# oss0430/SRFRD

Measured on AMD Instinct MI355X. Metric: sequences/sec, higher is better.
Workload: dtype f32

## Files before the change

srfrd_amd/csrc/srfrd_encoder_bwd_ragged_kernel.inc:

```
namespace SRFRD_NS {


struct RagBwdLds {
  lds_f* base;
  lds_f* s_ln;
  lds_f* s_lng;
};

template <int K_, int DI_, bool RMW_>
__device__ __forceinline__ void rag_bwd_seq(const EncArgs& a, const RagBwdLds& m, int b, int iter, int& tid, int wave, uint32_t seed) {
  const Dims& ly = a.dm;
  constexpr int nw = 8, nthr = 512;
  constexpr int L = 50, D = 50, LP = 64, DK = 52, DS = 54, NT = 4, MT = 4;
  constexpr int R = 52, SZ = R * DS, SLD = R + 2, SH = kRagSH;
  static_assert(SH == LP - R && R * SLD <= SZ + 2 * R, "slot geometry");
  static_assert(kRagBwdWork == SH * DS + 6 * SZ + 13 * LP, "working set");
  constexpr bool CV2 = true;
  constexpr int CIT = (R * (D / 2) + nthr - 1) / nthr;
  constexpr int PIT = (R * (R / 2) + nthr - 1) / nthr;
  lds_f* slot[6];
#pragma unroll
  for (int s = 0; s < 6; ++s) slot[s] = m.base + SH * DS + s * SZ;
  lds_f* tail = m.base + SH * DS + 6 * SZ;
  lds_i* s_in = (lds_i*)tail;
  lds_f* s_keep = tail + LP;
  lds_i* s_pid = (lds_i*)(tail + 2 * LP);
  lds_i* s_nid = (lds_i*)(tail + 3 * LP);
  lds_i* s_fk = (lds_i*)(tail + 4 * LP);
  lds_i* s_pfk = (lds_i*)(tail + 5 * LP);
  lds_i* s_nfk = (lds_i*)(tail + 6 * LP);
  lds_f* s_dpl = tail + 7 * LP;
  lds_f* s_dnl = tail + 8 * LP;
  lds_f* s_delta = tail + 9 * LP;
  lds_f* s_brep = tail + 10 * LP;
  lds_f* s_dummy = tail + 11 * LP;
  lds_f* s_misc = tail + 12 * LP;
  lds_f* s_ln = m.s_ln;
  lds_f* s_lng = m.s_lng;
  const float* P = a.dense;
  const bool drop_on = a.drop_on != 0;
  const int rkind = K_ >= 0 ? K_ : ly.kind;
  const bool is_sas = rkind == SRFRD_SASREC;
  const bool has_fake = rkind == SRFRD_SRFR || rkind == SRFRD_SRFRN;
  const bool is_srfu = rkind >= SRFRD_SRFU_B;
  constexpr int di = DI_, dfk = D - DI_;
  constexpr int dout = (K_ == SRFRD_SRFR) ? DI_ : D;
  const float sqrtD = sqrtf((float)di);
  const float qscale = a.qscale;
  const int B = a.B;
  auto pk = [&](int mat, int form) {
    return PackedB{reinterpret_cast<const float4*>(a.packed) + ((int64_t)mat * 2 + form) * (kPackFloats / 4)};
  };
  static_assert(L <= nthr && (R - L) * DS <= nthr, "single-pass helpers");
  auto ones_col = [&](lds_f* buf) {
    if (tid < L) buf[tid * DS + D] = 1.0f;
  };
  auto zero_pad_rows = [&](lds_f* buf) {
    if (tid < (R - L) * DS) buf[L * DS + tid] = 0.f;
  };
  const float keep_scale = drop_on ? a.drop_scale : 1.0f;

  asm volatile("" : "+v"(tid));
  float* slab = a.grad_slabs + (int64_t)blockIdx.x * ly.n_dense;
  const int rmw = RMW_ ? (iter != 0) : 0;
  if (iter == 0)
    for (int i = tid; i < ly.blk0; i += nthr) slab[i] = 0.f;
  const int64_t rowbase = (int64_t)b * L;
  const uint32_t seq = (uint32_t)(a.seq0 + b);
  const int lane0 = tid & 63;
  if (tid < LP) {
    const int t = tid;
    const bool in = t < L;
    const int id = in ? clamp_id(a.in_ids[rowbase + t], ly.n_items) : 0;
    const int pid = (in && a.pos_ids) ? clamp_id(a.pos_ids[rowbase + t], ly.n_items) : 0;
    const int nid = (in && a.neg_ids) ? clamp_id(a.neg_ids[rowbase + t], ly.n_items) : 0;
    s_in[t] = id;
    s_keep[t] = id != 0 ? 1.f : 0.f;
    s_pid[t] = pid;
    s_nid[t] = nid;
    s_fk[t] = (in && a.fk_ids) ? clamp_id(a.fk_ids[rowbase + t], 2) : 0;
    s_pfk[t] = (in && a.pos_fk) ? clamp_id(a.pos_fk[rowbase + t], 2) : 0;
    s_nfk[t] = (in && a.neg_fk) ? clamp_id(a.neg_fk[rowbase + t], 2) : 0;
    float dp = 0.f, dn = 0.f;
    if (in) {
      if (a.fused_bce) {
        const float pl = a.c_pl[rowbase + t], nl = a.c_nl[rowbase + t];
        if (pid != 0) {
          dp = sigmoid_f(pl) - 1.0f;
          dn = sigmoid_f(nl);
        }
      } else {
        if (a.d_pos && a.pos_ids) dp = a.d_pos[rowbase + t];
        if (a.d_neg && a.neg_ids) dn = a.d_neg[rowbase + t];
      }
    }
    s_dpl[t] = dp;
    s_dnl[t] = dn;
  }
  if (is_srfu && wave == 1) {
    const int lab = user_label_wave(rkind, a.fk_ids ? a.fk_ids + rowbase : nullptr, L, ly.n_labels);
    if (lane0 == 0) ((lds_i*)s_misc)[0] = lab;
  }
  __syncthreads();
  int t0, th;
  {
    const bool inr = lane0 < L;
    const unsigned long long nz = __ballot(inr && s_in[lane0] != 0);
    const unsigned long long ng = __ballot(inr && (s_in[lane0] != 0 || s_dpl[lane0] != 0.f || s_dnl[lane0] != 0.f));
    t0 = nz ? (int)__builtin_ctzll(nz) : L;
    th = ng ? (int)__builtin_ctzll(ng) : L;
    if (a.ragged_off) t0 = 0;
    if (a.d_hidden != nullptr || a.ragged_off) th = 0;
    t0 = __builtin_amdgcn_readfirstlane(t0);
    th = __builtin_amdgcn_readfirstlane(th);
  }
  const int krp = t0 >= 1 ? t0 - 1 : 0;
  const int kr = krp + SH, v0 = t0 + SH;
  const int mt0 = kr >> 4, r0 = mt0 << 4, mtn = MT - mt0;
  const int p0 = r0 > SH ? r0 - SH : 0;
  const int k0 = p0 + SH;
  const int hp = th < krp ? th : krp;
  const int mh0 = (hp + SH) >> 4, rh0 = mh0 << 4, mhn = MT - mh0;
  const int ph0 = rh0 > SH ? rh0 - SH : 0, kh0 = ph0 + SH;

  lds_f *sX = slot[0], *sQ = slot[1], *sG = slot[2], *sT = slot[3], *sK = slot[4], *sO = slot[5];
  lds_f* dummy = s_dummy;
#define TB(p) ((p) - SH * DS)
  G2L<CIT, CV2> g_last, g_h1, g_r;
  g_last.load(a.c_save_x + x_off(ly.n_blocks, b, ly.n_blocks, L, D) + p0 * D, L - p0, D, nthr);
  g_h1.load(a.c_save_h1 + h1_off(ly.n_blocks - 1, b, ly.n_blocks, L, D) + p0 * D, L - p0, D, nthr);
  g_r.load(a.c_save_aux + aux_off(ly.n_blocks - 1, b, ly.n_blocks, L, LP, D).r + p0 * D, L - p0, D, nthr);
  g_last.store(sX + p0 * DS, DS, L - p0, D, nthr);
  for (int r = ph0 + (tid >> 6); r < p0; r += nthr >> 6) {
    const int c = tid & 63;
    if (c < DS && c != D) sX[r * DS + c] = 0.f;
  }
  zero_pad_rows(sX);
  ones_col(sX);
  zero_pad_rows(sG);
  __syncthreads();

  int lane = tid & 63, li = lane & 15, lq = lane >> 4;
#define RG_RELANE() do { asm volatile("" : "+v"(tid)); lane = tid & 63; li = lane & 15; lq = lane >> 4; } while (0)
  const int nt_w = wave & 3, g_w = wave >> 2;
  auto slab_gemm = [&](int kk0, auto amat, auto bmat, const SlabWB& sl, const SlabPre& pre) {
    f32x4 acc[2];
#pragma unroll
    for (int j = 0; j < 2; ++j) acc[j] = f32x4{pre.v[j][0], pre.v[j][1], pre.v[j][2], pre.v[j][3]};
    mma_group<2>(acc, amat, bmat, (g_w << 4) + li, 32, (nt_w << 4) + li, kk0, LP, lq);
    const SlabCol sc = slab_col(sl, (nt_w << 4) + li);
    if (sc.ok) {
#pragma unroll
      for (int j = 0; j < 2; ++j)
#pragma unroll
        for (int e = 0; e < 4; ++e) {
          const int r = ((g_w + 2 * j) << 4) + (lq << 2) + e;
          if (r < sl.R) sl.base[(unsigned)(sc.col0 + r * sc.rs)] = acc[j][e];
        }
    }
  };
  auto col_sums = [&](int kk0, const lds_f* m_b, lds_f* dst, int ncol) {
    if (wave < NT) {
      f32x4 acc[1] = {f32x4{0.f, 0.f, 0.f, 0.f}};
      mma_group<1>(acc, OnesRow{}, Mat{m_b, DS}, li, 0, (wave << 4) + li, kk0, LP, lq);
      const int c = (wave << 4) + li;
      if (lq == 0 && c < ncol) dst[c] += acc[0][0];
    }
  };
  auto side_sums = [&](int n_out, auto term, auto dst_off, int tlo) {
    for (int p = wave; p < n_out; p += nw) {
      float sacc = 0.f;
      for (int t = tlo + lane; t < L; t += 64) sacc += term(p, t);
      sacc = wave_sum(sacc);
      if (lane == 0) atomicAdd(&slab[dst_off(p)], sacc);
    }
  };

  const lds_f* lnin = sX;
  if (K_ == SRFRD_SRFR) {
    const WFrag wl = load_wfrag(pk(ly.n_blocks * 6, 0), P + ly.off_lc_b, di, (di + 15) >> 4, tid);
    {
      constexpr int nst = (di + 15) >> 4;
      const int nt3 = wave % nst, g3 = wave / nst;
      auto epi = [&](int r, int c, float v) { *((c < di && r >= SH && r < SH + L) ? &TB(sQ)[r * DS + c] : dummy + c) = v; };
      if (g3 < 2) {
        if (g3 + 2 < mhn) gemm_group_packed<2>(mh0 + g3, 2, nt3, DK >> 2, Mat{TB(sX), DS}, wl, epi, lane);
        else if (g3 < mhn) gemm_group_packed<1>(mh0 + g3, 2, nt3, DK >> 2, Mat{TB(sX), DS}, wl, epi, lane);
      }
    }
    __syncthreads();
    lnin = sQ;
  }
  {
    const bool srfrn = K_ == SRFRD_SRFRN;
    const int n = (L - ph0) * dout;
    constexpr int GIT = (LP * D + nthr - 1) / nthr;
    constexpr int HALF = (GIT + 1) / 2;
    const float* hid = a.c_hidden + (rowbase + ph0) * dout;
    const float* dhid = a.d_hidden ? a.d_hidden + (rowbase + ph0) * dout : nullptr;
    int tg = tid;
    asm volatile("" : "+v"(tg));
    auto chunks = [&](auto bf16_shadow) {
      constexpr bool H16 = decltype(bf16_shadow)::value;
      for (int base0 = 0; base0 < n; base0 += HALF * nthr) {
        float hv[HALF], pv[HALF], nv[HALF];
#pragma unroll
        for (int u = 0; u < HALF; ++u) {
          const int i = min(base0 + u * nthr + tg, n - 1);
          const int tt = i / dout, c = i - tt * dout, t = ph0 + tt;
          const bool item = c < di;
          const int prow = item ? s_pid[t] : s_pfk[t], nrow = item ? s_nid[t] : s_nfk[t];
          const int w = item ? di : dfk, cc = item ? c : c - di;
          const bool use = item || srfrn;
          hv[u] = hid[i];
          if constexpr (H16) {
            const float* side = P + ly.off_side;
            const float ps = side[(use && !item) ? prow * dfk + cc : 0], ns = side[(use && !item) ? nrow * dfk + cc : 0];
            const uint16_t ph = a.table16[item ? (int64_t)prow * di + cc : 0], nh = a.table16[item ? (int64_t)nrow * di + cc : 0];
            pv[u] = item ? bf16_to_f32(ph) : ps;
            nv[u] = item ? bf16_to_f32(nh) : ns;
          } else {
            const float* src = item ? a.table : P + ly.off_side;
            pv[u] = src[use ? (int64_t)prow * w + cc : 0];
            nv[u] = src[use ? (int64_t)nrow * w + cc : 0];
          }
        }
#pragma unroll
        for (int u = 0; u < HALF; ++u) {
          const int i = base0 + u * nthr + tg;
          if (i < n) {
            const int tt = i / dout, c = i - tt * dout, t = ph0 + tt;
            float dh = dhid ? dhid[i] : 0.f;
            if (c < di || srfrn) dh += s_dpl[t] * pv[u] + s_dnl[t] * nv[u];
            sT[t * DS + c] = hv[u];
            sG[t * DS + c] = dh;
          }
        }
      }
    };
    if (a.table16 != nullptr) chunks(std::true_type{});
    else chunks(std::false_type{});
    if (dout < D)
      for (int idx = tid; idx < (L - ph0) * (D - dout); idx += nthr) {
        const int tt = idx / (D - dout), cc = dout + idx - tt * (D - dout);
        sG[(ph0 + tt) * DS + cc] = 0.f;
      }
  }
  __syncthreads();
  {
    int t = ph0 + tid / di, c = tid - (tid / di) * di;
    constexpr int dt = nthr / di, dc = nthr - dt * di;
    for (; t < L;) {
      const float h = sT[t * DS + c];
      const float dp = s_dpl[t], dn = s_dnl[t];
      const int pid = s_pid[t], nid = s_nid[t];
      if (a.contrib != nullptr) {
        a.contrib[(((int64_t)0 * B + b) * L + t) * di + c] = pid != 0 ? dp * h : 0.f;
        a.contrib[(((int64_t)1 * B + b) * L + t) * di + c] = nid != 0 ? dn * h : 0.f;
      } else {
        if (pid != 0 && dp != 0.f) atomicAdd(&a.grad_table[(int64_t)pid * di + c], dp * h);
        if (nid != 0 && dn != 0.f) atomicAdd(&a.grad_table[(int64_t)nid * di + c], dn * h);
      }
      t += dt; c += dc;
      if (c >= di) { c -= di; ++t; }
    }
    if (a.contrib != nullptr)
      for (int idx = tid; idx < ph0 * di; idx += nthr) {
        a.contrib[(((int64_t)0 * B + b) * L) * di + idx] = 0.f;
        a.contrib[(((int64_t)1 * B + b) * L) * di + idx] = 0.f;
      }
  }
  if (K_ == SRFRD_SRFRN)
    side_sums(2 * dfk, [&](int p, int t) {
      constexpr int dq = dfk > 0 ? dfk : 1;
      const int f = 1 + p / dq, c = p - (f - 1) * dq;
      const float w = (s_pfk[t] == f ? s_dpl[t] : 0.f) + (s_nfk[t] == f ? s_dnl[t] : 0.f);
      return w * sT[t * DS + di + c];
    }, [&](int p) { return ly.off_side + dfk + p; }, ph0);
  ln_bwd_rows<false>(nw, sG + ph0 * DS, lnin + ph0 * DS, sK + ph0 * DS, sO + ph0 * DS, L - ph0, R - ph0, DS, dout,
                     s_ln + (4 * ly.n_blocks) * 64);
  if (dout < D)
    for (int idx = tid; idx < (L - ph0) * (D - dout); idx += nthr) {
      const int tt = idx / (D - dout), cc = dout + idx - tt * (D - dout);
      sK[(ph0 + tt) * DS + cc] = 0.f;
    }
  zero_pad_rows(sK);
  __syncthreads();
  col_sums(kh0, TB(sG), s_lng + (4 * ly.n_blocks + 1) * 64, dout);
  col_sums(kh0, TB(sO), s_lng + (4 * ly.n_blocks + 0) * 64, dout);
  __syncthreads();
  lds_f* G = sK;
  lds_f* fr[5] = {sG, sO, sT, sQ, sX};
  if (K_ == SRFRD_SRFR) {
    {
      const SlabWB sl{slab, ly.off_lc_w, ly.off_lc_b, di, D, rmw};
      SlabPre pre = RMW_ ? slab_preload(nw, NT, NT, sl) : SlabPre{};
      slab_gemm(kh0, MatT{TB(G), DS}, Mat{TB(sX), DS}, sl, pre);
    }
    const WFrag wln = load_wfrag(pk(ly.n_blocks * 6, 1), nullptr, 0, NT, tid);
    lds_f* Gn = sG;
    {
      auto epi = [&](int r, int c, float v) { *((c < D && r >= SH) ? &TB(Gn)[r * DS + c] : dummy + c) = v; };
      if (g_w + 2 < mhn) gemm_group_packed<2>(mh0 + g_w, 2, nt_w, ((di + 3) & ~3) >> 2, Mat{TB(G), DS}, wln, epi, lane);
      else if (g_w < mhn) gemm_group_packed<1>(mh0 + g_w, 2, nt_w, ((di + 3) & ~3) >> 2, Mat{TB(G), DS}, wln, epi, lane);
    }
    __syncthreads();
    fr[0] = G;
    G = Gn;
  }

  for (int i = ly.n_blocks - 1; i >= 0; --i) {
    const BlkOff o = blk_off(ly.blk0 + i * ly.blk_stride, D);
    const DropSite ds2 = drop_site(drop_on, seed, site_ffn2(i), seq, a.drop_thr, a.drop_scale);
    const AuxOff ax = aux_off(i, b, ly.n_blocks, L, LP, D);
    RG_RELANE();
    lds_f *X = fr[0], *Rr = fr[1], *N = fr[2], *A2 = fr[3], *A1 = fr[4];
    launder(G); launder(X); launder(Rr); launder(N); launder(A2); launder(A1);
    const WFrag w2n = load_wfrag(pk(i * 6 + 5, 1), nullptr, 0, NT, tid);
    const SlabWB sl_w2{slab, o.c2_w, o.c2_b, D, D, rmw};
    const SlabWB sl_w1{slab, o.c1_w, o.c1_b, D, D, rmw};
    {
      const int c = tid & 63;
      if (c < D)
        for (int r = p0 + (tid >> 6); r < R; r += nthr >> 6) {
          const float g = r < L ? G[r * DS + c] * s_keep[r] : 0.f;
          if (r < L) G[r * DS + c] = g;
          A2[r * DS + c] = g * drop_mul(ds2, r, c);
        }
    }
    g_h1.store(X + p0 * DS, DS, L - p0, D, nthr);
    g_r.store(Rr + p0 * DS, DS, L - p0, D, nthr);
    zero_pad_rows(X); zero_pad_rows(Rr); zero_pad_rows(G);
    ones_col(Rr);
    __syncthreads();
    ln_rows(nw, X + p0 * DS, N + p0 * DS, L - p0, DS, D, s_ln + (4 * i + 2) * 64, s_ln + (4 * i + 3) * 64);
    zero_pad_rows(N);
    ones_col(N);
    __syncthreads();
    G2L<CIT, CV2> g_o, g_v, g_k;
    {
      SlabPre pre_w2 = RMW_ ? slab_preload(nw, NT, NT, sl_w2) : SlabPre{};
      rag_packed(mt0, mtn, DK >> 2, D, Mat{TB(A2), DS}, w2n, [&](int r, int c) { return TB(Rr)[r * DS + c]; },
                 [&](int r, int c, float v, float act) {
        *(r >= SH ? &TB(A1)[r * DS + c] : dummy + c) = act > 0.f ? v * keep_scale : 0.f;
      }, lane, wave);
      slab_gemm(k0, MatT{TB(A2), DS}, Mat{TB(Rr), DS}, sl_w2, pre_w2);
    }
    const WFrag w1n = load_wfrag(pk(i * 6 + 4, 1), nullptr, 0, NT, tid);
    g_o.load(a.c_save_aux + ax.o + p0 * D, L - p0, D, nthr);
    __syncthreads();
    {
      SlabPre pre_w1 = RMW_ ? slab_preload(nw, NT, NT, sl_w1) : SlabPre{};
      rag_packed(mt0, mtn, DK >> 2, D, Mat{TB(A1), DS}, w1n, [&](int r, int c) { return TB(G)[r * DS + c]; },
                 [&](int r, int c, float v, float old) { *(r >= SH ? &TB(G)[r * DS + c] : dummy + c) = old + v; }, lane, wave);
      slab_gemm(k0, MatT{TB(A1), DS}, Mat{TB(N), DS}, sl_w1, pre_w1);
    }
    g_v.load(a.c_save_aux + ax.v + p0 * D, L - p0, D, nthr);
    __syncthreads();
    lds_f *H = A2, *GX = Rr;
    ln_bwd_rows<false>(nw, G + p0 * DS, X + p0 * DS, H + p0 * DS, GX + p0 * DS, L - p0, R - p0, DS, D, s_ln + (4 * i + 2) * 64);
    zero_pad_rows(H);
    g_k.load(a.c_save_aux + ax.k + p0 * D, L - p0, D, nthr);
    __syncthreads();
    lds_f* O = N;
    col_sums(k0, TB(G), s_lng + (4 * i + 3) * 64, D);
    col_sums(k0, TB(GX), s_lng + (4 * i + 2) * 64, D);
    g_o.store(O + p0 * DS, DS, L - p0, D, nthr);
    zero_pad_rows(O);
    ones_col(O);
    const WFrag won = load_wfrag(pk(i * 6 + 3, 1), nullptr, 0, NT, tid);
    G2L<PIT, true> g_p;
    g_p.load2d(a.c_save_aux + ax.p + p0 * LP + p0, L - p0, R - p0, LP, nthr);
    float brep_v = 0.f;
    if (tid < L && tid >= t0 && t0 >= 1) brep_v = a.c_save_aux[ax.p + tid * LP + LP - 1];
    __syncthreads();
    lds_f *DO = G, *V = GX, *Kk = X, *S = A1;
    RG_RELANE();
    const SlabWB sl_wo{slab, o.out_w, o.out_b, D, D, rmw};
    G2L<CIT, CV2> g_q, g_x;
    {
      SlabPre pre_wo = RMW_ ? slab_preload(nw, NT, NT, sl_wo) : SlabPre{};
      g_v.store(V + p0 * DS, DS, L - p0, D, nthr);
      g_k.store(Kk + p0 * DS, DS, L - p0, D, nthr);
      zero_pad_rows(V); zero_pad_rows(Kk);
      rag_packed(mt0, mtn, DK >> 2, DK, Mat{TB(H), DS}, won, NoPre{},
                 [&](int r, int c, float v, float) { *(r >= SH ? &TB(DO)[r * DS + c] : dummy + c) = v; }, lane, wave);
      slab_gemm(k0, MatT{TB(H), DS}, Mat{TB(O), DS}, sl_wo, pre_wo);
    }
    g_q.load(a.c_save_aux + ax.q + p0 * D, L - p0, D, nthr);
    __syncthreads();
    {
      const int q = tid & (kRL - 1);
      for (int r = p0 + tid / kRL; r < L; r += nthr / kRL) {
        float s = 0.f;
#pragma unroll
        for (int j = 0; j < kQC; ++j) {
          const int c = q + kRL * j;
          if (c < D) s += DO[r * DS + c] * O[r * DS + c];
        }
        s = row_sum(s);
        if (q == 0) s_delta[r] = s;
// ... 220 lines not shown
```

srfrd_amd/csrc/srfrd_encoder_fwd_ragged_kernel.inc:

```
namespace SRFRD_NS {

constexpr int kRagSH = 12;

constexpr int kRagChunks = 2;
struct RagT0 {
  int v[kRagChunks];
};
__device__ __forceinline__ bool rag_ordered(const EncArgs& a) { return a.sched != nullptr && a.sched_mode != 0 && a.B <= 512 * kRagChunks; }
__device__ __forceinline__ RagT0 rag_load_t0(const EncArgs& a, int tid) {
  RagT0 t;
#pragma unroll
  for (int c = 0; c < kRagChunks; ++c) {
    const int b = c * 512 + tid;
    t.v[c] = (rag_ordered(a) && c * 512 < a.B) ? a.sched[kSchedT0 + min(b, a.B - 1)] : 0;
  }
  return t;
}

__device__ __forceinline__ int rag_select(const RagT0& t0v, int B, int want, lds_i* scr, int tid) {
  lds_i* hist = scr;
  lds_i* wcnt = scr + 64;
  lds_i* res = scr + 80;
  const int lane = tid & 63, wave = tid >> 6;
  constexpr int NCH = kRagChunks;
// ... 147 lines not shown
template <int G, class AL, class EPI, class POST>
__device__ __forceinline__ void rgemm_packed_dual(int mt, int mstride_tiles, int nt, int ksteps, int ncols, const AL& a, const WFrag& w1,
                                                  const WFrag& w2, const EPI& epi, int lane, const POST& post) {
  const int li = lane & 15, lq = lane >> 4;
  const int c = (nt << 4) + li;
  f32x4 acc1[G], acc2[G];
#pragma unroll
  for (int j = 0; j < G; ++j) { acc1[j] = f32x4{0.f, 0.f, 0.f, 0.f}; acc2[j] = f32x4{0.f, 0.f, 0.f, 0.f}; }
  const int mrow = (mt << 4) + li, mstride = mstride_tiles << 4;
  float av[4][G];
#pragma unroll
  for (int s = 0; s < 4; ++s)
    if (s < ksteps)
#pragma unroll
      for (int j = 0; j < G; ++j) av[s][j] = a(mrow + j * mstride, 4 * s + lq);
#pragma unroll
  for (int kc = 0; kc < kPackKC; ++kc) {
    const int nst = ksteps - 4 * kc;
    if (nst > 0) {
      const int nnext = nst - 4;
      float an[4][G];
#pragma unroll
      for (int s = 0; s < 4; ++s)
        if (s < nnext)
#pragma unroll
          for (int j = 0; j < G; ++j) an[s][j] = a(mrow + j * mstride, ((kc + 1) << 4) + 4 * s + lq);
      __builtin_amdgcn_sched_barrier(0);
#pragma unroll
      for (int s = 0; s < 4; ++s)
        if (s < nst)
#pragma unroll
          for (int j = 0; j < G; ++j) {
            acc1[j] = __builtin_amdgcn_mfma_f32_16x16x4f32(av[s][j], w1.q[kc][s], acc1[j], 0, 0, 0);
            acc2[j] = __builtin_amdgcn_mfma_f32_16x16x4f32(av[s][j], w2.q[kc][s], acc2[j], 0, 0, 0);
          }
      __builtin_amdgcn_sched_barrier(0);
#pragma unroll
      for (int s = 0; s < 4; ++s)
#pragma unroll
        for (int j = 0; j < G; ++j) av[s][j] = an[s][j];
    }
  }
  if (c < ncols) {
#pragma unroll
    for (int j = 0; j < G; ++j) {
      const int rb = ((mt + j * mstride_tiles) << 4) + (lq << 2);
      float g1[4], g2[4];
#pragma unroll
      for (int e = 0; e < 4; ++e) {
        g1[e] = acc1[j][e] + w1.bias;
        g2[e] = acc2[j][e] + w2.bias;
        epi(rb + e, c, g1[e], g2[e]);
      }
      post(rb, c, g1, g2);
    }
  }
}
template <class AL, class EPI, class POST>
__device__ __forceinline__ void rag_packed_dual(int m0, int mtn, int ksteps, int ncols, const AL& a, const WFrag& w1, const WFrag& w2,
                                                const EPI& epi, int lane, int wave, const POST& post) {
  const int nt = wave & 3, g = wave >> 2;
  if (g + 2 < mtn) rgemm_packed_dual<2>(m0 + g, 2, nt, ksteps, ncols, a, w1, w2, epi, lane, post);
  else if (g < mtn) rgemm_packed_dual<1>(m0 + g, 2, nt, ksteps, ncols, a, w1, w2, epi, lane, post);
}

typedef __attribute__((address_space(3))) f32x2 lds_f2r;
__device__ __forceinline__ void rag_softmax(lds_f* S, int rq0, int r0, int v0, int kr, int t0, int row_end, const DropSite& ds,
                                            float* gsave, int tid) {
  constexpr int LP = 64, SLD = 66, SH = kRagSH;
  const int m8 = (tid & 7) << 3;
  const int r = rq0 + (tid >> 3);
  if (r >= LP) return;
  lds_f2r* row2 = reinterpret_cast<lds_f2r*>(S + r * SLD + SH + m8);
  const bool own = m8 < 56;
  const int npair = m8 == 48 ? 2 : 4;
  const int ip = r - SH;
  float4* g4 = (gsave != nullptr && own && ip >= 0 && r < row_end) ? reinterpret_cast<float4*>(gsave + ip * LP + m8) : nullptr;
  if (r < v0 || r >= row_end) {
    if (own) {
#pragma unroll
      for (int i = 0; i < 4; ++i)
        if (i < npair) row2[i] = f32x2{0.f, 0.f};
    }
    if (g4 != nullptr) { g4[0] = make_float4(0.f, 0.f, 0.f, 0.f); g4[1] = make_float4(0.f, 0.f, 0.f, 0.f); }
    return;
  }
  const bool rep = t0 >= 1;
  const int krp = kr - SH;
  float x[8];
  if (own) {
#pragma unroll
    for (int i = 0; i < 4; ++i) { const f32x2 t = row2[i < npair ? i : 0]; x[2 * i] = t.x; x[2 * i + 1] = t.y; }
  }
  float mx = -INFINITY;
#pragma unroll
  for (int i = 0; i < 8; ++i) {
    const int pj = m8 + i;
    x[i] = (own && pj >= krp && pj <= ip) ? x[i] : -INFINITY;
    mx = fmaxf(mx, x[i]);
  }
  mx = row_max(mx);
  float s = 0.f;
#pragma unroll
  for (int i = 0; i < 8; ++i) {
    const int pj = m8 + i;
    const float e = (own && pj >= krp && pj <= ip) ? __expf(x[i] - mx) : 0.f;
    x[i] = e;
    s += (rep && pj == krp) ? e * (float)t0 : e;
  }
  s = row_sum(s);
  const float inv = 1.0f / s;
  float cnt = (float)t0;
  if (ds.on && rep) {
    int c = 0;
    for (int jj = tid & 7; jj < t0; jj += 8) c += drop_mul(ds, ip, jj) != 0.f ? 1 : 0;
    cnt = row_sum((float)c);
  }
  if (!own) return;
  const float scale = ds.on ? ds.scale : 1.0f;
  float pv[8], gs[8];
#pragma unroll
  for (int i = 0; i < 8; ++i) {
    const int pj = m8 + i;
    const float p = x[i] * inv;
    if (rep && pj == krp) {
      const float pm = p * cnt;
      if (gsave != nullptr) gsave[ip * LP + LP - 1] = p * (float)t0;
      pv[i] = pm * scale;
      gs[i] = pm;
    } else {
      const float mul = drop_mul(ds, ip, pj);
      pv[i] = p * mul;
      gs[i] = mul != 0.f ? p : -p;
    }
  }
#pragma unroll
  for (int i = 0; i < 4; ++i)
    if (i < npair) row2[i] = f32x2{pv[2 * i], pv[2 * i + 1]};
  if (g4 != nullptr) {
    g4[0] = make_float4(gs[0], gs[1], gs[2], gs[3]);
    g4[1] = make_float4(gs[4], gs[5], gs[6], gs[7]);
  }
}

struct RagFwdLds {
  lds_f *bXS, *bQN, *bQ, *bK, *bV;
  lds_i* s_in;
  lds_f* s_keep;
  lds_i *s_pid, *s_nid;
  lds_f* s_misc;
  lds_f* s_ln;
};

template <int K_, int T_, int DI_>
__device__ __forceinline__ void rag_fwd_seq(const EncArgs& a, const RagFwdLds& m, int b, int& tid, int wave, uint32_t seed) {
  const Dims& ly = a.dm;
  constexpr int D = 50, L = 50, LP = 64, DK = 52, DS = 54, SLD = 66, NT = 4, MT = 4, SH = kRagSH;
  constexpr int nw = 8, nthr = 512;
  static_assert(SH + L <= LP && (SH & 3) == 0, "tile coordinates");
  const int lane0 = threadIdx.x & 63;
  lds_f* bXS = m.bXS;
  lds_f* bQN = m.bQN;
  lds_f* bQ = m.bQ;
  lds_f* bK = m.bK;
  lds_f* bV = m.bV;
  lds_i* s_in = m.s_in;
  lds_f* s_keep = m.s_keep;
  lds_i* s_pid = m.s_pid;
  lds_i* s_nid = m.s_nid;
  lds_f* s_misc = m.s_misc;
  lds_f* s_ln = m.s_ln;
  const float* P = a.dense;
  const ItemTable table{a.table, a.table16};
  constexpr bool TR_ = T_ != 0;
  const bool has_pos = TR_ || a.pos_ids != nullptr, has_neg = TR_ || a.neg_ids != nullptr;
  const bool drop_on = TR_ || a.drop_on != 0, do_save = TR_ || a.save_x != nullptr, do_loss = TR_ || a.loss_part != nullptr;
  const int kind = K_ >= 0 ? K_ : ly.kind;
  const bool is_sas = kind == SRFRD_SASREC;
  const bool has_fake = kind == SRFRD_SRFR || kind == SRFRD_SRFRN;
  const bool is_srfu = kind >= SRFRD_SRFU_B;
  constexpr int di = DI_, dfk = D - DI_;
  constexpr int dout = (K_ == SRFRD_SRFR) ? DI_ : D;
  const float sqrtD = sqrtf((float)di);
  const float qscale = a.qscale;
  auto pk = [&](int mat, int form) {
    return PackedB{reinterpret_cast<const float4*>(a.packed) + ((int64_t)mat * 2 + form) * (kPackFloats / 4)};
  };

  asm volatile("" : "+v"(tid));
  const int64_t rowbase = (int64_t)b * L;
  const uint32_t seq = (uint32_t)(a.seq0 + b);
  if (tid < LP) {
    const int t = tid - SH;
    const bool in = t >= 0 && t < L;
    const int id = in ? clamp_id(a.in_ids[rowbase + t], ly.n_items) : 0;
    s_in[tid] = id;
    s_keep[tid] = id != 0 ? 1.f : 0.f;
    s_pid[tid] = (in && has_pos) ? clamp_id(a.pos_ids[rowbase + t], ly.n_items) : 0;
    s_nid[tid] = (in && has_neg) ? clamp_id(a.neg_ids[rowbase + t], ly.n_items) : 0;
  }
  if (is_srfu && wave == 1) {
    const int lab = user_label_wave(kind, a.fk_ids ? a.fk_ids + rowbase : nullptr, L, ly.n_labels);
    if (lane0 == 0) ((lds_i*)s_misc)[0] = lab;
  }
  __syncthreads();
  int v0;
  {
    const unsigned long long nz = __ballot(s_in[tid & 63] != 0);
    v0 = nz ? (int)__builtin_ctzll(nz) : SH + L;
    if (a.ragged_off) v0 = SH;
    v0 = __builtin_amdgcn_readfirstlane(v0);
  }
  const int t0 = v0 - SH;
  const int kr = t0 >= 1 ? v0 - 1 : v0;
  const int mt0 = kr >> 4, r0 = mt0 << 4, mtn = MT - mt0;
  const int tstart = r0 > SH ? r0 - SH : 0;

  {
    const DropSite dsE = drop_site(drop_on && is_sas, seed, SITE_EMB, seq, a.drop_thr, a.drop_scale);
    const int lab = is_srfu ? ((lds_i*)s_misc)[0] : 0;
    if (r0 < SH)
      for (int i = tid; i < (SH - r0) * DS; i += nthr) bXS[r0 * DS + i] = 0.f;
    for (int i = tid; i < (LP - SH - L) * DS; i += nthr) bXS[(SH + L) * DS + i] = 0.f;
    int t = tstart + tid / D, c = tid - (tid / D) * D;
    constexpr int dt = nthr / D, dc = nthr - dt * D;
    for (; t < L;) {
      const int id = s_in[t + SH];
      float v;
      if (has_fake) {
        if (c < di) v = table((int64_t)id * di + c) + P[ly.off_pos + t * di + c];
        else v = P[ly.off_side + ((a.fk_ids ? clamp_id(a.fk_ids[rowbase + t], 2) : 0)) * dfk + (c - di)];
      } else {
        v = table((int64_t)id * di + c);
        if (is_sas) v *= sqrtD;
        v += P[ly.off_pos + t * di + c];
        if (is_srfu) v += P[ly.off_side + lab * D + c];
        if (is_sas) v *= drop_mul(dsE, t, c);
      }
      v *= s_keep[t + SH];
      bXS[(t + SH) * DS + c] = v;
      if (do_save) a.save_x[x_off(0, b, ly.n_blocks, L, D) + t * D + c] = v;
      t += dt; c += dc;
      if (c >= D) { c -= D; ++t; }
    }
  }
  __syncthreads();

  for (int i = 0; i < ly.n_blocks; ++i) {
    const BlkOff o = blk_off(ly.blk0 + i * ly.blk_stride, D);
    launder(bXS); launder(bQN); launder(bQ); launder(bK); launder(bV);
    asm volatile("" : "+v"(tid));
    const int lane = tid & 63;
    const bool lo = !TR_ && a.last_only != 0 && i == ly.n_blocks - 1;
    const int mq0 = lo ? (L - 1 + SH) >> 4 : mt0, rq0 = mq0 << 4, mqn = MT - mq0;
    const AuxOff ax = aux_off(i, b, ly.n_blocks, L, LP, D, 1);
    float* sv_r = do_save ? a.save_aux + ax.r : nullptr;
    float* sv_o = do_save ? a.save_aux + ax.o : nullptr;
    float* sv_p = do_save ? a.save_aux + ax.p : nullptr;
    float* sv_q = do_save ? a.save_aux + ax.q : nullptr;
    float* sv_k = do_save ? a.save_aux + ax.k : nullptr;
    float* sv_v = do_save ? a.save_aux + ax.v : nullptr;
    auto gstore4 = [&](float* plane, int rb, int c, const float (&v)[4]) {
      const int p0 = rb - SH;
      const unsigned off = (unsigned)(p0 * D + c);
      if (p0 >= 0 && p0 + 3 < L) {
        plane[off] = v[0]; plane[off + D] = v[1]; plane[off + 2 * D] = v[2]; plane[off + 3 * D] = v[3];
      } else {
#pragma unroll
        for (int e = 0; e < 4; ++e)
          if ((unsigned)(p0 + e) < (unsigned)L) plane[(unsigned)((p0 + e) * D + c)] = v[e];
      }
    };
    const WFrag wq = load_wfrag(pk(i * 6 + 0, 0), P + o.in_b, D, NT, tid);
    const WFrag wk = load_wfrag(pk(i * 6 + 1, 0), P + o.in_b + D, D, NT, tid);
    const WFrag wv = load_wfrag(pk(i * 6 + 2, 0), P + o.in_b + 2 * D, D, NT, tid);
    ln_rows(nw, bXS + rq0 * DS, bQN + rq0 * DS, LP - rq0, DS, D, s_ln + (4 * i + 0) * 64, s_ln + (4 * i + 1) * 64);
    __syncthreads();
    rag_packed(mq0, mqn, DK >> 2, D, Mat{bQN, DS}, wq, NoPre{}, [&](int r, int c, float v, float) {
      bQ[r * DS + c] = v * qscale;
      return v * qscale;
    }, lane, wave, [&](int rb, int c, const float (&gv)[4]) { if (sv_q) gstore4(sv_q, rb, c, gv); });
    rag_packed_dual(mt0, mtn, DK >> 2, D, Mat{bXS, DS}, wk, wv, [&](int r, int c, float vk, float vv) {
      bK[r * DS + c] = vk;
      bV[r * DS + c] = vv;
    }, lane, wave, [&](int rb, int c, const float (&gk)[4], const float (&gv)[4]) {
      if (sv_k) { gstore4(sv_k, rb, c, gk); gstore4(sv_v, rb, c, gv); }
    });
    const WFrag wo = load_wfrag(pk(i * 6 + 3, 0), P + o.out_b, D, NT, tid);
    const WFrag w1 = load_wfrag(pk(i * 6 + 4, 0), P + o.c1_b, D, NT, tid);
    __syncthreads();
    {
      const int li = lane & 15, lq = lane >> 4;
      if (lo) {
        for (int u = wave; u < mtn; u += nw)
          gemm_group<0, 1>(0, 1, u << 4, DK, Mat{bQ + rq0 * DS, DS}, MatT{bK + r0 * DS, DS},
                           [&](int r, int c, float v) { bXS[(r + rq0) * SLD + c + r0] = v; }, li, lq);
      } else {
        const int ntri = (mtn * (mtn + 1)) >> 1;
        for (int u = wave; u < ntri; u += nw) {
          const int m = u >= 6 ? 3 : (u >= 3 ? 2 : (u >= 1 ? 1 : 0)), n = u - ((m * (m + 1)) >> 1);
          gemm_group<0, 1>(m, 1, n << 4, DK, Mat{bQ + r0 * DS, DS}, MatT{bK + r0 * DS, DS},
                           [&](int r, int c, float v) { bXS[(r + r0) * SLD + c + r0] = v; }, li, lq);
        }
      }
    }
    __syncthreads();
    {
      const DropSite dsA = drop_site(drop_on, seed, site_attn(i), seq, a.drop_thr, a.drop_scale);
      rag_softmax(bXS, rq0, r0, v0, kr, t0, SH + L, dsA, sv_p, tid);
    }
    __syncthreads();
    {
      const int li = lane & 15, lq = lane >> 4;
      const int nt = wave & 3, g = wave >> 2;
      auto epi_o = [&](int r_, int c, float v) {
        const int r = r_ + rq0;
        if (c < D) {
          bQ[r * DS + c] = v;
          if (sv_o && (unsigned)(r - SH) < (unsigned)L) sv_o[(unsigned)((r - SH) * D + c)] = v;
        }
      };
      if (lo) {
        if (g == 0) {
          const int kk0 = r0 > SH ? r0 : SH;
          gemm_group<0, 1>(0, 1, nt << 4, LP - kk0, Mat{bXS + rq0 * SLD + kk0, SLD}, Mat{bV + kk0 * DS, DS}, epi_o, li, lq);
        }
      } else {
        const int kk0 = r0 > SH ? r0 : SH;
        const Mat Ap{bXS + r0 * SLD + kk0, SLD};
        const Mat Bv{bV + kk0 * DS, DS};
        const int kend = LP - kk0;
        int ma, mb;
        if (mtn == 4) { ma = g == 0 ? 0 : 1; mb = g == 0 ? 3 : 2; }
        else if (mtn == 3) { ma = g == 0 ? 2 : 0; mb = g == 0 ? -1 : 1; }
        else if (mtn == 2) { ma = g == 0 ? 1 : 0; mb = -1; }
        else { ma = g == 0 ? 0 : -1; mb = -1; }
        if (ma >= 0) gemm_group<2, 1>(ma, 1, nt << 4, kend, Ap, Bv, epi_o, li, lq);
        if (mb >= 0) gemm_group<2, 1>(mb, 1, nt << 4, kend, Ap, Bv, epi_o, li, lq);
      }
    }
    __syncthreads();
    rag_packed(mq0, mqn, DK >> 2, D, Mat{bQ, DS}, wo, [&](int r, int c) { return bQN[r * DS + c]; }, [&](int r, int c, float v, float res) {
      const float h = res + v;
      bXS[r * DS + c] = h;
      return h;
    }, lane, wave, [&](int rb, int c, const float (&gv)[4]) { if (do_save) gstore4(a.save_h1 + h1_off(i, b, ly.n_blocks, L, D), rb, c, gv); });
    __syncthreads();
    ln_rows(nw, bXS + rq0 * DS, bQN + rq0 * DS, LP - rq0, DS, D, s_ln + (4 * i + 2) * 64, s_ln + (4 * i + 3) * 64);
    __syncthreads();
    const DropSite ds1 = drop_site(drop_on, seed, site_ffn1(i), seq, a.drop_thr, a.drop_scale);
    const DropSite ds2 = drop_site(drop_on, seed, site_ffn2(i), seq, a.drop_thr, a.drop_scale);
    const WFrag w2 = load_wfrag(pk(i * 6 + 5, 0), P + o.c2_b, D, NT, tid);
    rag_packed(mq0, mqn, DK >> 2, D, Mat{bQN, DS}, w1, NoPre{}, [&](int r, int c, float v, float) {
      const float h = fmaxf(v * drop_mul(ds1, r - SH, c), 0.f);
      bQ[r * DS + c] = h;
      return h;
    }, lane, wave, [&](int rb, int c, const float (&gv)[4]) { if (sv_r) gstore4(sv_r, rb, c, gv); });
    __syncthreads();
    rag_packed(mq0, mqn, DK >> 2, D, Mat{bQ, DS}, w2, [&](int r, int c) { return bQN[r * DS + c]; }, [&](int r, int c, float v, float res) {
      const float y = (v * drop_mul(ds2, r - SH, c) + res) * s_keep[r];
      bXS[r * DS + c] = y;
      return y;
    }, lane, wave, [&](int rb, int c, const float (&gv)[4]) { if (do_save) gstore4(a.save_x + x_off(i + 1, b, ly.n_blocks, L, D), rb, c, gv); });
    __syncthreads();
  }

  const bool lo_h = !TR_ && a.last_only != 0;
  asm volatile("" : "+v"(tid));
  const int lane = tid & 63;
  if (!lo_h && r0 > SH) {
    for (int i = tid; i < (r0 - SH) * DS; i += nthr) bXS[SH * DS + i] = 0.f;
    __syncthreads();
  }
  lds_f* xp = bXS + SH * DS;
  lds_f* qnp = bQN + SH * DS;
  const lds_f* hin = xp;
  const int p0h = lo_h ? L - 1 : 0;
  if (kind == SRFRD_SRFR) {
    const WFrag wl = load_wfrag(pk(ly.n_blocks * 6, 0), P + ly.off_lc_b, di, (di + 15) >> 4, tid);
    const int mh0 = lo_h ? MT - 1 : 0;
    {
      constexpr int nst = (di + 15) >> 4;
      const int nt = wave % nst, g = wave / nst;
      const int mtn_h = MT - mh0;
      auto epi = [&](int r_, int c, float v) { if (c < di) bQ[(r_ + (mh0 << 4)) * DS + c] = v; };
      if (g < 2) {
        if (g + 2 < mtn_h) gemm_group_packed<2>(g, 2, nt, DK >> 2, Mat{bXS + (mh0 << 4) * DS, DS}, wl, epi, lane);
        else if (g < mtn_h) gemm_group_packed<1>(g, 2, nt, DK >> 2, Mat{bXS + (mh0 << 4) * DS, DS}, wl, epi, lane);
      }
    }
    __syncthreads();
    hin = bQ + SH * DS;
  }
  ln_rows(nw, hin + p0h * DS, qnp + p0h * DS, L - p0h, DS, dout, s_ln + (4 * ly.n_blocks) * 64, s_ln + (4 * ly.n_blocks + 1) * 64);
  __syncthreads();
  if (lo_h) {
    for (int c = tid; c < dout; c += nthr) a.hidden[(int64_t)b * dout + c] = qnp[(L - 1) * DS + c];
  } else {
    const bool srfrn = kind == SRFRD_SRFRN;
    lds_f* kp = bK + SH * DS;
    lds_f* vp = bV + SH * DS;
    {
      int t = tid / dout, c = tid - t * dout;
      constexpr int dt = nthr / dout, dc = nthr - dt * dout;
      for (; t < L;) {
        const float h = qnp[t * DS + c];
        a.hidden[(rowbase + t) * dout + c] = h;
        if (has_pos)
          kp[t * DS + c] = h * (c < di ? table((int64_t)s_pid[t + SH] * di + c)
                                       : (srfrn ? P[ly.off_side + clamp_id(a.pos_fk[rowbase + t], 2) * dfk + (c - di)] : 0.f));
        if (has_neg)
          vp[t * DS + c] = h * (c < di ? table((int64_t)s_nid[t + SH] * di + c)
                                       : (srfrn ? P[ly.off_side + clamp_id(a.neg_fk[rowbase + t], 2) * dfk + (c - di)] : 0.f));
        t += dt; c += dc;
        if (c >= dout) { c -= dout; ++t; }
      }
    }
    __syncthreads();
    float sp = 0.f, sn = 0.f, cnt = 0.f;
    const int q = tid & (kRL - 1);
    for (int t = tid / kRL; t < L; t += nthr / kRL) {
      float ap = 0.f, an = 0.f;
#pragma unroll
      for (int j = 0; j < kQC; ++j) {
        const int c = q + kRL * j;
        if (c < dout) {
          if (has_pos) ap += kp[t * DS + c];
          if (has_neg) an += vp[t * DS + c];
        }
      }
      const float pl = row_sum(ap), nl = row_sum(an);
      if (q == 0) {
        if (has_pos) a.pos_logits[rowbase + t] = pl;
        if (has_neg) a.neg_logits[rowbase + t] = nl;
        if (do_loss && s_pid[t + SH] != 0) {
          sp += softplus_fast(-pl);
          sn += softplus_fast(nl);
          cnt += 1.f;
        }
      }
    }
    if (do_loss) {
      sp = wave_sum(sp); sn = wave_sum(sn); cnt = wave_sum(cnt);
      if (lane == 0) {
        s_misc[8 + wave * 3 + 0] = sp;
        s_misc[8 + wave * 3 + 1] = sn;
        s_misc[8 + wave * 3 + 2] = cnt;
      }
      __syncthreads();
      if (tid < 3) {
        float s = 0.f;
        for (int w = 0; w < nw; ++w) s += s_misc[8 + w * 3 + tid];
        a.loss_part[(int64_t)b * 3 + tid] = s;
      }
    }
  }
  __syncthreads();
}

template <int K_, int T_, int DI_>
__global__ void __launch_bounds__(512, 4) encoder_fwd_ragged_kernel(const EncArgs a) {
  extern __shared__ __attribute__((aligned(16))) float smem[];
  const Dims& ly = a.dm;
  constexpr int D = 50, L = 50, LP = 64, DS = 54, SLD = 66;
  constexpr int nthr = 512;
  int tid = threadIdx.x;
  const int wave = __builtin_amdgcn_readfirstlane(tid >> 6);
  constexpr int szA = LP * DS, szX = LP * SLD;
  const int tailsz = 4 * LP + 64 + ln_cache_floats(ly.n_blocks);
  const RagT0 t0v = rag_load_t0(a, tid);
  lds_f* c_cur = (lds_f*)smem;
  auto carve = [&](int64_t n) -> lds_f* { lds_f* p = c_cur; c_cur += n; return p; };
  {
    Geom g = make_geom(L, D);
    const int total = (int)fwd_lds_floats(g, ly.n_blocks);
    for (int i = tid; i < total; i += nthr) ((lds_f*)smem)[i] = 0.f;
  }
  lds_f* tail = carve(tailsz);
  RagFwdLds m;
  m.bXS = carve(szX);
  m.bQN = carve(szA);
  m.bQ = carve(szA);
  m.bK = carve(szA);
  m.bV = carve(szA + kSlack);
  m.s_in = (lds_i*)tail;
  m.s_keep = tail + LP;
  m.s_pid = (lds_i*)(tail + 2 * LP);
  m.s_nid = (lds_i*)(tail + 3 * LP);
  m.s_misc = tail + 4 * LP;
  lds_f* s_ln = m.s_misc + 64;
  m.s_ln = s_ln;
  __syncthreads();
  fill_ln_cache(s_ln, a.dense, ly);
  const uint32_t seed = a.seed_dev ? *a.seed_dev : a.seed;

  STAMP_INIT
  for (int iter = 0;; ++iter) {
    const int b = __builtin_amdgcn_readfirstlane(rag_take(a, (lds_i*)m.bXS, iter, tid, t0v));
    if (b < 0) break;
    rag_fwd_seq<K_, T_, DI_>(a, m, b, tid, wave, seed);
  }
}

}
```

srfrd_amd/csrc/srfrd_encoder_train_ragged.hip:

```cpp
#include "srfrd_enc_common.h"

#include "srfrd_encoder_fwd_ragged_kernel.inc"
#include "srfrd_encoder_bwd_ragged_kernel.inc"

namespace srfrd {

template <int K_, int DI_, bool RMW_>
__global__ void __launch_bounds__(512, 4) encoder_train_ragged_kernel(const EncArgs a) {
  extern __shared__ __attribute__((aligned(16))) float smem[];
  const Dims& ly = a.dm;
  constexpr int LP = 64, DS = 54, SLD = 66, nthr = 512;
  constexpr int W = kRagFwdWork > kRagBwdWork ? kRagFwdWork : kRagBwdWork;
  int tid = threadIdx.x;
  const int wave = __builtin_amdgcn_readfirstlane(tid >> 6);
  const RagT0 t0v = rag_load_t0(a, tid);
  lds_f* base = (lds_f*)smem;
  {
    const int total = (int)train_ragged_lds_floats(ly.n_blocks);
    for (int i = tid; i < total; i += nthr) base[i] = 0.f;
  }
  RagFwdLds fm;
  fm.bXS = base;
  fm.bQN = base + LP * SLD;
  fm.bQ = fm.bQN + LP * DS;
  fm.bK = fm.bQ + LP * DS;
  fm.bV = fm.bK + LP * DS;
  lds_f* ftail = fm.bV + LP * DS;
  fm.s_in = (lds_i*)ftail;
  fm.s_keep = ftail + LP;
  fm.s_pid = (lds_i*)(ftail + 2 * LP);
  fm.s_nid = (lds_i*)(ftail + 3 * LP);
  fm.s_misc = ftail + 4 * LP;
  static_assert(LP * SLD + 4 * LP * DS + 5 * LP == kRagFwdWork, "forward working set");
  lds_f* s_ln = base + W;
  fm.s_ln = s_ln;
  const RagBwdLds bm{base, s_ln, s_ln + ln_cache_floats(ly.n_blocks)};
  __syncthreads();
  fill_ln_cache(s_ln, a.dense, ly);
  const uint32_t seed = a.seed_dev ? *a.seed_dev : a.seed;

  for (int iter = 0;; ++iter) {
    if (iter > 0) {
      for (int i = tid; i < W; i += nthr) base[i] = 0.f;
      __syncthreads();
    }
    const int b = __builtin_amdgcn_readfirstlane(rag_take(a, (lds_i*)fm.bXS, iter, tid, t0v));
    if (b < 0) break;
    rag_fwd_seq<K_, 1, DI_>(a, fm, b, tid, wave, seed);
    for (int i = tid; i < W; i += nthr) base[i] = 0.f;
    __syncthreads();
    rag_bwd_seq<K_, DI_, RMW_>(a, bm, b, iter, tid, wave, seed);
  }
}

int launch_train_ragged(const KernelPlan& k, const EncArgs& a, void* stream) {
  return with_variant(k.variant, [&](auto v) {
    constexpr KindVariant kv = kKindVariants[decltype(v)::value];
    return with_flag(k.flag, [&](auto rmw) { return launch_enc(encoder_train_ragged_kernel<kv.K, kv.DI, decltype(rmw)::value>, k, stream, a); });
  });
}

}

using namespace srfrd;

extern "C" int srfrd_encoder_train_sched(const srfrd_layout* lay, const void* item_table, const float* dense, const float* packed,
                                         const int64_t* input_ids, const int64_t* fake_ids, const int64_t* pos_ids,
                                         const int64_t* pos_fake, const int64_t* neg_ids, const int64_t* neg_fake, int B, int L,
                                         double dropout_p, uint32_t seed, const uint32_t* seed_dev, int64_t seq_index0,
                                         float* hidden, float* pos_logits, float* neg_logits, float* save_x, float* save_h1,
                                         float* save_aux, float* loss_part, const float* d_hidden, const float* d_pos,
                                         const float* d_neg, int fused_bce, float* grad_table, float* table_contrib,
                                         float* grad_slabs, float* scratch, int64_t scratch_floats, const int32_t* sched,
                                         int sched_mode, void* stream) {
  if (sched_mode < 0 || sched_mode > 1 || (sched_mode != 0 && !sched)) return SRFRD_E_ARG;
  const int sw = read_switches();
  EncArgs a = {};
  a.sched = sched_mode != 0 ? sched : nullptr;
  a.sched_mode = a.sched ? sched_mode : 0;
  a.ragged_off = (sw & SRFRD_SW_RAGGED_FULL_ROWS) != 0;
  const int rc = fill_args(a, lay, item_table, dense, packed, input_ids, fake_ids, pos_ids, pos_fake, neg_ids, neg_fake, B, L,
                           dropout_p, seed, seed_dev, seq_index0);
  if (rc) return rc;
  if (!hidden || (pos_ids && !pos_logits) || (neg_ids && !neg_logits)) return SRFRD_E_ARG;
  if (loss_part && !(pos_ids && neg_ids)) return SRFRD_E_ARG;
  if ((save_x != nullptr) != (save_h1 != nullptr) || (save_x != nullptr) != (save_aux != nullptr)) return SRFRD_E_ARG;
  if (!save_x || !grad_table || !grad_slabs) return SRFRD_E_ARG;
  if (fused_bce && !(pos_ids && neg_ids)) return SRFRD_E_ARG;
  const int mode = (pos_ids ? SRFRD_PLAN_POS : 0) | (neg_ids ? SRFRD_PLAN_NEG : 0) | SRFRD_PLAN_CKPT | (loss_part ? SRFRD_PLAN_LOSS : 0) |
                   (dropout_p > 0.0 ? SRFRD_PLAN_DROPOUT : 0) | (fused_bce && !d_hidden ? SRFRD_PLAN_FUSED_BCE : 0);
  const KernelPlan k = encoder_plan(*lay, B, L, mode, sw, num_cu(), scratch ? scratch_floats : 0).train;
  if (k.rc) return k.rc;
  a.hidden = hidden; a.pos_logits = pos_logits; a.neg_logits = neg_logits;
  a.save_x = save_x; a.save_h1 = save_h1; a.save_aux = save_aux; a.loss_part = loss_part;
  a.c_hidden = hidden; a.c_pl = pos_logits; a.c_nl = neg_logits; a.c_save_x = save_x; a.c_save_h1 = save_h1; a.c_save_aux = save_aux;
  a.fused_bce = 1;
  a.grad_table = grad_table; a.grad_slabs = grad_slabs; a.contrib = table_contrib;
  return launch_train_ragged(k, a, stream);
}
```

Before: 2.949 million.

## Hand forward LDS state directly to backward in fused ragged training kernel

For SASRec-style kinds with full item width, the training kernel now passes the forward pass's LDS buffers (final hidden, gathered pos/neg item rows, logits, ids) straight into the backward pass. It no longer reloads saved activations, logits and ids from global memory, and it skips the full-workspace zeroing pass between the two phases. The forward stores raw item rows and applies the product inside the logit reduction. The backward builds the hidden gradient from LDS with explicit rounding so results match the old path. Only the needed LDS regions are zeroed, using 16-byte stores. The cost is tight coupling of the two LDS layouts, held together by hard-coded offset asserts, plus some extra registers.

Result: faster. 3.078 million (median of 6 runs) (+4.4%).

```diff
diff --git a/srfrd_amd/csrc/srfrd_encoder_bwd_ragged_kernel.inc b/srfrd_amd/csrc/srfrd_encoder_bwd_ragged_kernel.inc
--- a/srfrd_amd/csrc/srfrd_encoder_bwd_ragged_kernel.inc
+++ b/srfrd_amd/csrc/srfrd_encoder_bwd_ragged_kernel.inc
@@ -7,8 +7,25 @@
   lds_f* s_lng;
 };
 
-template <int K_, int DI_, bool RMW_>
-__device__ __forceinline__ void rag_bwd_seq(const EncArgs& a, const RagBwdLds& m, int b, int iter, int& tid, int wave, uint32_t seed) {
+__device__ __forceinline__ void rag_bce_grad(int pid, float pl, float nl, float& dp, float& dn) {
+  dp = 0.f; dn = 0.f;
+  if (pid != 0) {
+    dp = sigmoid_f(pl) - 1.0f;
+    dn = sigmoid_f(nl);
+  }
+}
+__device__ __forceinline__ float rag_dh(float dh0, float dp, float pv, float dn, float nv) {
+  float p1 = __fmul_rn(dp, pv), p2 = __fmul_rn(dn, nv);
+  asm("" : "+v"(p1));
+  asm("" : "+v"(p2));
+  float s1 = __fadd_rn(p1, dh0);
+  asm("" : "+v"(s1));
+  return __fadd_rn(s1, p2);
+}
+
+template <int K_, int DI_, bool RMW_, bool SEAM_ = false>
+__device__ __forceinline__ void rag_bwd_seq(const EncArgs& a, const RagBwdLds& m, int b, int iter, int& tid, int wave, uint32_t seed,
+                                            const RagFwdLds* f = nullptr) {
   const Dims& ly = a.dm;
   constexpr int nw = 8, nthr = 512;
   constexpr int L = 50, D = 50, LP = 64, DK = 52, DS = 54, NT = 4, MT = 4;
@@ -68,6 +85,19 @@
   const int64_t rowbase = (int64_t)b * L;
   const uint32_t seq = (uint32_t)(a.seq0 + b);
   const int lane0 = tid & 63;
+  static_assert(!SEAM_ || kRagSeam<K_, DI_>, "the seam covers plain item-row heads only");
+  int sm_id = 0, sm_pid = 0, sm_nid = 0, sm_lab = 0;
+  float sm_dp = 0.f, sm_dn = 0.f;
+  if constexpr (SEAM_) {
+    const bool in = lane0 < L;
+    const int tr = min(lane0 + SH, LP - 1);
+    sm_id = in ? f->s_in[tr] : 0;
+    sm_pid = in ? f->s_pid[tr] : 0;
+    sm_nid = in ? f->s_nid[tr] : 0;
+    const float pl = f->bQ[lane0], nl = f->bQ[LP + lane0];
+    if (in) rag_bce_grad(sm_pid, pl, nl, sm_dp, sm_dn);
+    if (is_srfu) sm_lab = ((lds_i*)f->s_misc)[0];
+  } else {
   if (tid < LP) {
     const int t = tid;
     const bool in = t < L;
@@ -85,10 +115,7 @@
     if (in) {
       if (a.fused_bce) {
         const float pl = a.c_pl[rowbase + t], nl = a.c_nl[rowbase + t];
-        if (pid != 0) {
-          dp = sigmoid_f(pl) - 1.0f;
-          dn = sigmoid_f(nl);
-        }
+        rag_bce_grad(pid, pl, nl, dp, dn);
       } else {
         if (a.d_pos && a.pos_ids) dp = a.d_pos[rowbase + t];
         if (a.d_neg && a.neg_ids) dn = a.d_neg[rowbase + t];
@@ -102,11 +129,18 @@
     if (lane0 == 0) ((lds_i*)s_misc)[0] = lab;
   }
   __syncthreads();
+  }
   int t0, th;
   {
     const bool inr = lane0 < L;
-    const unsigned long long nz = __ballot(inr && s_in[lane0] != 0);
-    const unsigned long long ng = __ballot(inr && (s_in[lane0] != 0 || s_dpl[lane0] != 0.f || s_dnl[lane0] != 0.f));
+    unsigned long long nz, ng;
+    if constexpr (SEAM_) {
+      nz = __ballot(inr && sm_id != 0);
+      ng = __ballot(inr && (sm_id != 0 || sm_dp != 0.f || sm_dn != 0.f));
+    } else {
+      nz = __ballot(inr && s_in[lane0] != 0);
+      ng = __ballot(inr && (s_in[lane0] != 0 || s_dpl[lane0] != 0.f || s_dnl[lane0] != 0.f));
+    }
     t0 = nz ? (int)__builtin_ctzll(nz) : L;
     th = ng ? (int)__builtin_ctzll(ng) : L;
     if (a.ragged_off) t0 = 0;
@@ -126,7 +160,72 @@
   lds_f *sX = slot[0], *sQ = slot[1], *sG = slot[2], *sT = slot[3], *sK = slot[4], *sO = slot[5];
   lds_f* dummy = s_dummy;
 #define TB(p) ((p) - SH * DS)
-  G2L<CIT, CV2> g_last, g_h1, g_r;
+  G2L<CIT, CV2> g_h1, g_r;
+  if constexpr (SEAM_) {
+    constexpr int NE = (L * D + nthr - 1) / nthr;
+    constexpr int oX = SH * DS, oG = oX + 2 * SZ, oT = oX + 3 * SZ, oTail = oX + 6 * SZ;
+    static_assert(DS == 54 && D == DI_ && NE * nthr >= L * D, "row stride of both kernels; every element has a thread");
+    static_assert(oG == 6264 && oT == 9072 && oTail == 17496 && kRagBwdWork == 18328, "backward layout");
+    static_assert(LP * 66 + SH * DS == 4872 && LP * 66 + 2 * LP * DS + SH * DS == 11784 && LP * 66 + 3 * LP * DS + SH * DS == 15240,
+                  "forward layout: qnp, kp, vp");
+    static_assert((oX % 4) == 0 && ((oX + L * DS) % 4) == 0 && (oG % 4) == 0 && ((oT + SZ) % 4) == 0 && (oTail % 4) == 0,
+                  "16-byte zero stores");
+    const lds_f* qnp = f->bQN + SH * DS;
+    const lds_f* kp = f->bK + SH * DS;
+    const lds_f* vp = f->bV + SH * DS;
+    float zero = 0.f;
+    asm("" : "+v"(zero));
+    float hv[NE], dhv[NE];
+#pragma unroll
+    for (int u = 0; u < NE; ++u) {
+      const int i = min(u * nthr + tid, L * D - 1);
+      const int t = i / D, c = i - t * D;
+      hv[u] = qnp[t * DS + c];
+      dhv[u] = rag_dh(zero, __shfl(sm_dp, t, 64), kp[t * DS + c], __shfl(sm_dn, t, 64), vp[t * DS + c]);
+    }
+    g_h1.load(a.c_save_h1 + h1_off(ly.n_blocks - 1, b, ly.n_blocks, L, D) + p0 * D, L - p0, D, nthr);
+    g_r.load(a.c_save_aux + aux_off(ly.n_blocks - 1, b, ly.n_blocks, L, LP, D).r + p0 * D, L - p0, D, nthr);
+    __syncthreads();
+    {
+      typedef __attribute__((address_space(3))) f32x4 lds_f4;
+      lds_f4* z4 = (lds_f4*)m.base;
+      constexpr int a0 = oX / 4, b0 = (oX + L * DS) / 4, b1 = oG / 4, c0 = (oT + SZ) / 4, c1 = oTail / 4;
+      constexpr int n4 = a0 + (b1 - b0) + (c1 - c0);
+      for (int i = tid; i < n4; i += nthr) {
+        const int j = i < a0 ? i : (i < a0 + (b1 - b0) ? i - a0 + b0 : i - a0 - (b1 - b0) + c0);
+        z4[j] = f32x4{0.f, 0.f, 0.f, 0.f};
+      }
+    }
+    if (tid < L * (DS - D)) {
+      const int r = tid >> 2, c = D + (tid & 3);
+      static_assert(DS - D == 4, "four spare columns");
+      sX[r * DS + c] = c == D ? 1.0f : 0.f;
+      sG[r * DS + c] = 0.f;
+      sT[r * DS + c] = 0.f;
+    }
+    if (tid < (R - L) * DS) { sG[L * DS + tid] = 0.f; sT[L * DS + tid] = 0.f; }
+#pragma unroll
+    for (int u = 0; u < NE; ++u) {
+      const int i = u * nthr + tid;
+      if (i < L * D) {
+        const int t = i / D, c = i - t * D;
+        sT[t * DS + c] = t >= ph0 ? hv[u] : 0.f;
+        sG[t * DS + c] = t >= ph0 ? dhv[u] : 0.f;
+      }
+    }
+    if (wave == 0) {
+      s_in[lane0] = sm_id;
+      s_keep[lane0] = sm_id != 0 ? 1.f : 0.f;
+      s_pid[lane0] = sm_pid;
+      s_nid[lane0] = sm_nid;
+      s_fk[lane0] = 0; s_pfk[lane0] = 0; s_nfk[lane0] = 0;
+      s_dpl[lane0] = sm_dp;
+      s_dnl[lane0] = sm_dn;
+      s_delta[lane0] = 0.f; s_brep[lane0] = 0.f; s_dummy[lane0] = 0.f;
+      ((lds_i*)s_misc)[lane0] = lane0 == 0 ? sm_lab : 0;
+    }
+  } else {
+  G2L<CIT, CV2> g_last;
   g_last.load(a.c_save_x + x_off(ly.n_blocks, b, ly.n_blocks, L, D) + p0 * D, L - p0, D, nthr);
   g_h1.load(a.c_save_h1 + h1_off(ly.n_blocks - 1, b, ly.n_blocks, L, D) + p0 * D, L - p0, D, nthr);
   g_r.load(a.c_save_aux + aux_off(ly.n_blocks - 1, b, ly.n_blocks, L, LP, D).r + p0 * D, L - p0, D, nthr);
@@ -138,6 +237,7 @@
   zero_pad_rows(sX);
   ones_col(sX);
   zero_pad_rows(sG);
+  }
   __syncthreads();
 
   int lane = tid & 63, li = lane & 15, lq = lane >> 4;
@@ -191,6 +291,7 @@
     __syncthreads();
     lnin = sQ;
   }
+  if constexpr (!SEAM_) {
   {
     const bool srfrn = K_ == SRFRD_SRFRN;
     const int n = (L - ph0) * dout;
@@ -231,7 +332,8 @@
           if (i < n) {
             const int tt = i / dout, c = i - tt * dout, t = ph0 + tt;
             float dh = dhid ? dhid[i] : 0.f;
-            if (c < di || srfrn) dh += s_dpl[t] * pv[u] + s_dnl[t] * nv[u];
+            if constexpr (kRagSeam<K_, DI_>) dh = rag_dh(dh, s_dpl[t], pv[u], s_dnl[t], nv[u]);
+            else if (c < di || srfrn) dh += s_dpl[t] * pv[u] + s_dnl[t] * nv[u];
             sT[t * DS + c] = hv[u];
             sG[t * DS + c] = dh;
           }
@@ -247,6 +349,7 @@
       }
   }
   __syncthreads();
+  }
   {
     int t = ph0 + tid / di, c = tid - (tid / di) * di;
     constexpr int dt = nthr / di, dc = nthr - dt * di;
diff --git a/srfrd_amd/csrc/srfrd_encoder_fwd_ragged_kernel.inc b/srfrd_amd/csrc/srfrd_encoder_fwd_ragged_kernel.inc
--- a/srfrd_amd/csrc/srfrd_encoder_fwd_ragged_kernel.inc
+++ b/srfrd_amd/csrc/srfrd_encoder_fwd_ragged_kernel.inc
@@ -323,7 +323,16 @@
   lds_f* s_ln;
 };
 
-template <int K_, int T_, int DI_>
+template <int K_, int DI_>
+constexpr bool kRagSeam = (K_ == SRFRD_SASREC || K_ == -1) && DI_ == 50;
+
+__device__ __forceinline__ float rag_mul_rounded(float a, float b) {
+  float p = __fmul_rn(a, b);
+  asm("" : "+v"(p));
+  return p;
+}
+
+template <int K_, int T_, int DI_, bool SEAM_ = false>
 __device__ __forceinline__ void rag_fwd_seq(const EncArgs& a, const RagFwdLds& m, int b, int& tid, int wave, uint32_t seed) {
   const Dims& ly = a.dm;
   constexpr int D = 50, L = 50, LP = 64, DK = 52, DS = 54, SLD = 66, NT = 4, MT = 4, SH = kRagSH;
@@ -352,6 +361,7 @@
   const bool is_srfu = kind >= SRFRD_SRFU_B;
   constexpr int di = DI_, dfk = D - DI_;
   constexpr int dout = (K_ == SRFRD_SRFR) ? DI_ : D;
+  static_assert(!SEAM_ || (kRagSeam<K_, DI_> && TR_), "the seam: training forward of a kind whose head it covers");
   const float sqrtD = sqrtf((float)di);
   const float qscale = a.qscale;
   auto pk = [&](int mat, int form) {
@@ -577,12 +587,17 @@
       for (; t < L;) {
         const float h = qnp[t * DS + c];
         a.hidden[(rowbase + t) * dout + c] = h;
-        if (has_pos)
-          kp[t * DS + c] = h * (c < di ? table((int64_t)s_pid[t + SH] * di + c)
-                                       : (srfrn ? P[ly.off_side + clamp_id(a.pos_fk[rowbase + t], 2) * dfk + (c - di)] : 0.f));
-        if (has_neg)
-          vp[t * DS + c] = h * (c < di ? table((int64_t)s_nid[t + SH] * di + c)
-                                       : (srfrn ? P[ly.off_side + clamp_id(a.neg_fk[rowbase + t], 2) * dfk + (c - di)] : 0.f));
+        if constexpr (SEAM_) {
+          kp[t * DS + c] = table((int64_t)s_pid[t + SH] * di + c);
+          vp[t * DS + c] = table((int64_t)s_nid[t + SH] * di + c);
+        } else {
+          if (has_pos)
+            kp[t * DS + c] = h * (c < di ? table((int64_t)s_pid[t + SH] * di + c)
+                                         : (srfrn ? P[ly.off_side + clamp_id(a.pos_fk[rowbase + t], 2) * dfk + (c - di)] : 0.f));
+          if (has_neg)
+            vp[t * DS + c] = h * (c < di ? table((int64_t)s_nid[t + SH] * di + c)
+                                         : (srfrn ? P[ly.off_side + clamp_id(a.neg_fk[rowbase + t], 2) * dfk + (c - di)] : 0.f));
+        }
         t += dt; c += dc;
         if (c >= dout) { c -= dout; ++t; }
       }
@@ -596,12 +611,19 @@
       for (int j = 0; j < kQC; ++j) {
         const int c = q + kRL * j;
         if (c < dout) {
-          if (has_pos) ap += kp[t * DS + c];
-          if (has_neg) an += vp[t * DS + c];
+          if constexpr (SEAM_) {
+            const float h = qnp[t * DS + c];
+            ap += rag_mul_rounded(h, kp[t * DS + c]);
+            an += rag_mul_rounded(h, vp[t * DS + c]);
+          } else {
+            if (has_pos) ap += kp[t * DS + c];
+            if (has_neg) an += vp[t * DS + c];
+          }
         }
       }
       const float pl = row_sum(ap), nl = row_sum(an);
       if (q == 0) {
+        if constexpr (SEAM_) { bQ[t] = pl; bQ[LP + t] = nl; }
         if (has_pos) a.pos_logits[rowbase + t] = pl;
         if (has_neg) a.neg_logits[rowbase + t] = nl;
         if (do_loss && s_pid[t + SH] != 0) {
diff --git a/srfrd_amd/csrc/srfrd_encoder_train_ragged.hip b/srfrd_amd/csrc/srfrd_encoder_train_ragged.hip
--- a/srfrd_amd/csrc/srfrd_encoder_train_ragged.hip
+++ b/srfrd_amd/csrc/srfrd_encoder_train_ragged.hip
@@ -46,10 +46,15 @@
     }
     const int b = __builtin_amdgcn_readfirstlane(rag_take(a, (lds_i*)fm.bXS, iter, tid, t0v));
     if (b < 0) break;
-    rag_fwd_seq<K_, 1, DI_>(a, fm, b, tid, wave, seed);
-    for (int i = tid; i < W; i += nthr) base[i] = 0.f;
-    __syncthreads();
-    rag_bwd_seq<K_, DI_, RMW_>(a, bm, b, iter, tid, wave, seed);
+    constexpr bool SEAM = kRagSeam<K_, DI_>;
+    rag_fwd_seq<K_, 1, DI_, SEAM>(a, fm, b, tid, wave, seed);
+    if constexpr (SEAM) {
+      rag_bwd_seq<K_, DI_, RMW_, true>(a, bm, b, iter, tid, wave, seed, &fm);
+    } else {
+      for (int i = tid; i < W; i += nthr) base[i] = 0.f;
+      __syncthreads();
+      rag_bwd_seq<K_, DI_, RMW_>(a, bm, b, iter, tid, wave, seed);
+    }
   }
 }
 
```
